# g1mv/density

Measured on NVIDIA H100. Metric: chameleon_encode_input_GBps, higher is better.
Workload: dtype u32

## Files before the change

### density_b200/csrc/chameleon_encode.cu

```cuda
#include <cstdio>
#include "common.cuh"
#include "encode_internal.cuh"

namespace dns {
namespace cham {

constexpr int FP_THREADS = 1024;
constexpr int FP_QPT = 4;
constexpr int TILE_Q = FP_THREADS * FP_QPT;
constexpr int SIDE_N = 8192;
constexpr uint32_t SIDE_EMPTY = 0xFFFFFFFFu;

constexpr int CLS_N = 32;
constexpr int CLS_CAP = 128;

constexpr uint32_t R_TOUCHED = 1u << 12, R_SLOW = 1u << 13, R_FIRST = 1u << 14;

struct FlagSmem {
    uint16_t tab[65536];
    uint32_t vbit[2048];
    uint32_t conf[2048];
    uint32_t side[SIDE_N];
    uint2 rec[TILE_Q];
    uint16_t cls_list[CLS_N][CLS_CAP];
// ... 30 lines not shown
        const uint32_t q = qs[pos];
        const uint32_t p = hash_prod(q);
        const uint32_t hh = valid ? prod_hash(p) : 0x10000u + lane;
        const uint32_t ff = prod_fp(p, q);
        uint32_t cur = 0; bool touched = false;
        if (valid) { cur = S.tab[hh]; touched = cur != 0 || bit_test(S.vbit, hh); }
        const uint32_t grp = __match_any_sync(0xFFFFFFFFu, hh);
        const uint32_t lower = grp & lanemask_lt();
        const int pl = lower ? 31 - __clz(lower) : 0;
        const uint32_t fprev = __shfl_sync(0xFFFFFFFFu, ff, pl);
        const bool hit = valid && (lower ? (fprev == ff) : (touched && cur == ff));
        const bool is_last = (grp & lanemask_gt()) == 0;
        if (valid && is_last && (lower || !hit)) {
            S.tab[hh] = (uint16_t)ff;
            if (ff == 0) atomicOr(&S.vbit[hh >> 5], 1u << (hh & 31));
        }
        const uint32_t fb = __ballot_sync(0xFFFFFFFFu, hit);
        if (lane == 0) S.sigw[c] = fb;
        append_unres(valid && !lower && !touched, run_q0 + pos, hh, ff, &S.unres_count, unres_run);
        __syncwarp();
    }
}

__global__ void __launch_bounds__(FP_THREADS, 1)
cham_flag_pass(const uint32_t* __restrict__ in, uint64_t nquads, uint32_t tiles_total, uint32_t nruns,
               uint32_t* __restrict__ sigw_g,
               uint2* __restrict__ unres,
               uint32_t* __restrict__ unres_count,
               uint32_t* __restrict__ final_tab,
               const uint8_t* __restrict__ copymap,
               const Status* __restrict__ gate)
{
    if (gate && !(gate->nonquiet && !gate->converged)) return;
    extern __shared__ __align__(16) unsigned char smem_raw[];
    FlagSmem& S = *reinterpret_cast<FlagSmem*>(smem_raw);
    const uint32_t tid = threadIdx.x, lane = tid & 31, warp = tid >> 5;
    const uint32_t run = blockIdx.x;
    const uint64_t t_begin = (uint64_t)run * tiles_total / nruns;
    const uint64_t t_end = (uint64_t)(run + 1) * tiles_total / nruns;
    uint2* __restrict__ unres_run = unres + (size_t)run * 65536;
    const uint32_t pos0 = warp * 128 + lane;
    const uint32_t ntile_run = (uint32_t)(t_end - t_begin);
    const uint64_t q_begin = t_begin * TILE_Q;
    const uint64_t q_end64 = (t_end * TILE_Q < nquads) ? t_end * TILE_Q : nquads;
    const uint32_t run_quads = q_begin < q_end64 ? (uint32_t)(q_end64 - q_begin) : 0u;
    const uint32_t* __restrict__ rin = in + q_begin;
    uint32_t* __restrict__ rsig = sigw_g + t_begin * (TILE_Q / 32);
    const uint8_t* __restrict__ rcm = copymap ? copymap + t_begin * 64 : nullptr;

    {
        uint4 z = make_uint4(0, 0, 0, 0);
        uint4* t4 = reinterpret_cast<uint4*>(S.tab);
        #pragma unroll 1
        for (uint32_t i = tid; i < 65536 * 2 / 16; i += FP_THREADS) t4[i] = z;
        #pragma unroll 1
        for (uint32_t i = tid; i < 2048; i += FP_THREADS) { S.vbit[i] = 0; S.conf[i] = 0; }
        #pragma unroll 1
        for (uint32_t i = tid; i < SIDE_N; i += FP_THREADS) S.side[i] = SIDE_EMPTY;
        if (tid < CLS_N) S.cls_count[tid] = 0;
        if (tid == 0) { S.unres_count = 0; S.cls_overflow = 0; S.nrec = 0; }
    }
    __syncthreads();

    uint32_t nxt[FP_QPT];
#pragma unroll
    for (int j = 0; j < FP_QPT; ++j) nxt[j] = (pos0 + 32 * j < run_quads) ? ld_stream_u32(rin + pos0 + 32 * j) : 0u;

#ifdef DNS_PHASE_TIMING
    long long ph[8] = {0, 0, 0, 0, 0, 0, 0, 0}, tprev = clock64();
#define DNS_PH(k) { long long tn = clock64(); ph[k] += tn - tprev; tprev = tn; }
#else
#define DNS_PH(k)
#endif
    #pragma unroll 1
    for (uint32_t lt = 0; lt < ntile_run; ++lt) {
        uint32_t q[FP_QPT], h[FP_QPT], f[FP_QPT];
        const uint32_t run_q0 = lt * TILE_Q;
        const uint32_t left = run_q0 < run_quads ? run_quads - run_q0 : 0u;
        const uint32_t rem = left < (uint32_t)TILE_Q ? left : (uint32_t)TILE_Q;
#pragma unroll
        for (int j = 0; j < FP_QPT; ++j) q[j] = nxt[j];
        {
            const uint32_t nleft = left > (uint32_t)TILE_Q ? left - TILE_Q : 0u;
            const uint32_t* __restrict__ np = rin + run_q0 + TILE_Q + pos0;
#pragma unroll
            for (int j = 0; j < FP_QPT; ++j) nxt[j] = (pos0 + 32 * j < nleft) ? ld_stream_u32(np + 32 * j) : 0u;
        }

        uint32_t actmask = 0;
        {
            uint32_t cp = 0;
            if (rcm) cp = (rcm[lt * 64 + warp * 2] ? 1u : 0u) | (rcm[lt * 64 + warp * 2 + 1] ? 2u : 0u);
#pragma unroll
            for (int j = 0; j < FP_QPT; ++j)
                if (pos0 + 32 * j < rem && !((cp >> (j >> 1)) & 1u)) actmask |= 1u << j;
        }
        uint32_t missmask = 0;
        {
            uint32_t old[FP_QPT], tch = 0;
#pragma unroll
            for (int j = 0; j < FP_QPT; ++j) {
                const uint32_t p = hash_prod(q[j]);
                h[j] = prod_hash(p);
                f[j] = prod_fp(p, q[j]);
                old[j] = S.tab[h[j]];
            }
            uint32_t mb[FP_QPT], tot = 0;
#pragma unroll
            for (int j = 0; j < FP_QPT; ++j) {
                bool touched = old[j] != 0;
                if (!touched) touched = bit_test(S.vbit, h[j]);
                if (touched) tch |= 1u << j;
                const bool miss = ((actmask >> j) & 1u) && !(touched && old[j] == f[j]);
                if (miss) missmask |= 1u << j;
                mb[j] = __ballot_sync(0xFFFFFFFFu, miss);
                tot += __popc(mb[j]);
            }
            if (tot) {
                uint32_t base = 0;
                if (lane == 0) base = atomicAdd(&S.nrec, tot);
                base = __shfl_sync(0xFFFFFFFFu, base, 0);
#pragma unroll
                for (int j = 0; j < FP_QPT; ++j) {
                    if (missmask & (1u << j))
                        S.rec[base + __popc(mb[j] & lanemask_lt())] =
                            make_uint2(h[j] | (f[j] << 16), (pos0 + 32 * j) | ((tch >> j) & 1u ? R_TOUCHED : 0u) | (old[j] << 16));
                    base += __popc(mb[j]);
                }
            }
        }
        __syncthreads();
        DNS_PH(0)
        const uint32_t nmiss = S.nrec;

        #pragma unroll 1
        for (uint32_t i = tid; i < nmiss; i += FP_THREADS) {
            const uint2 r = S.rec[i];
            const uint32_t hh = r.x & 0xFFFFu;
            S.tab[hh] = (uint16_t)(r.x >> 16);
            atomicMin(&S.side[hh & (SIDE_N - 1)], ((r.y & 0xFFFu) << 16) | hh);
        }
        __syncthreads();
        DNS_PH(1)

#pragma unroll
        for (int j = 0; j < FP_QPT; ++j) {
            const uint32_t pos = pos0 + 32 * j;
            bool ok = false;
            if (((actmask >> j) & 1u) && !(missmask & (1u << j))) {
                ok = S.tab[h[j]] == f[j];
                if (!ok) {
                    const uint32_t slot = S.side[h[j] & (SIDE_N - 1)];
                    if ((slot & 0xFFFFu) == h[j] && pos < (slot >> 16)) {
                        ok = true;
                    } else {
                        const uint32_t idx = atomicAdd(&S.nrec, 1u);
                        S.rec[idx] = make_uint2(h[j] | (f[j] << 16), pos | R_TOUCHED | (f[j] << 16));
                        const uint32_t c = h[j] >> 11;
                        const uint32_t k = atomicAdd(&S.cls_count[c], 1u);
                        if (k < CLS_CAP) S.cls_list[c][k] = (uint16_t)idx; else S.cls_overflow = 1;
                        atomicOr(&S.conf[h[j] >> 5], 1u << (h[j] & 31));
                    }
                }
            }
            const uint32_t fb = __ballot_sync(0xFFFFFFFFu, ok);
            if (lane == 0) S.sigw[warp * 4 + j] = fb;
        }
        #pragma unroll 1
        for (uint32_t i = tid; i < nmiss; i += FP_THREADS) {
            const uint2 r = S.rec[i];
            const uint32_t hh = r.x & 0xFFFFu;
            const uint32_t slot = S.side[hh & (SIDE_N - 1)];
            const uint32_t w = S.tab[hh];
            uint32_t y = r.y;
            if ((slot & 0xFFFFu) != hh || w != (r.x >> 16)) {
                y |= R_SLOW;
                atomicOr(&S.conf[hh >> 5], 1u << (hh & 31));
            } else if (slot == (((r.y & 0xFFFu) << 16) | hh)) {
                y |= R_FIRST;
            }
            if (y != r.y) S.rec[i].y = y;
        }
        __syncthreads();
        DNS_PH(2)

        #pragma unroll 1
        for (uint32_t i = tid; i < nmiss; i += FP_THREADS) {
            const uint2 r = S.rec[i];
            const uint32_t hh = r.x & 0xFFFFu;
            uint32_t y = r.y;
            if (!(y & R_SLOW) && bit_test(S.conf, hh)) { y |= R_SLOW; S.rec[i].y = y; }
            if (y & R_SLOW) {
                const uint32_t c = hh >> 11;
                const uint32_t k = atomicAdd(&S.cls_count[c], 1u);
                if (k < CLS_CAP) S.cls_list[c][k] = (uint16_t)i; else S.cls_overflow = 1;
            } else if (!(y & R_FIRST)) {
                const uint32_t pos = y & 0xFFFu;
                atomicOr(&S.sigw[pos >> 5], 1u << (pos & 31));
            }
            S.side[hh & (SIDE_N - 1)] = SIDE_EMPTY;
        }
        __syncthreads();
        DNS_PH(3)

        S.conf[tid] = 0; S.conf[tid + FP_THREADS] = 0;
        if (S.cls_overflow) {
            #pragma unroll 1
            for (uint32_t i = tid; i < nmiss; i += FP_THREADS) {
                const uint2 r = S.rec[i];
                S.tab[r.x & 0xFFFFu] = (uint16_t)(r.y >> 16);
            }
            if (tid < CLS_N) S.cls_count[tid] = 0;
            __syncthreads();
            uint32_t* qs = reinterpret_cast<uint32_t*>(S.rec);
#pragma unroll
            for (int j = 0; j < FP_QPT; ++j) qs[pos0 + 32 * j] = q[j];
            if (tid == 0) { S.nrec = 0; S.cls_overflow = 0; }
            __syncthreads();
            if (warp == 0) tile_in_order(S, qs, rem, run_q0, unres_run, rcm ? rcm + lt * 64 : nullptr);
        } else {
            #pragma unroll 1
            for (uint32_t base = warp * 32; base < nmiss; base += FP_THREADS) {
                const uint32_t i = base + lane;
                uint2 r = make_uint2(0, 0);
                if (i < nmiss) r = S.rec[i];
                const uint32_t hh = r.x & 0xFFFFu;
                const bool first = (i < nmiss) && (r.y & (R_FIRST | R_SLOW)) == R_FIRST;
                if (first && (r.x >> 16) == 0) atomicOr(&S.vbit[hh >> 5], 1u << (hh & 31));
                append_unres(first && !(r.y & R_TOUCHED), run_q0 + (r.y & 0xFFFu), hh, r.x >> 16, &S.unres_count, unres_run);
            }
            const uint32_t n = S.cls_count[warp];
            const uint16_t* __restrict__ lst = S.cls_list[warp];
            #pragma unroll 1
            for (uint32_t base = 0; base < n; base += 32) {
                const uint32_t i = base + lane;
                const bool valid = i < n;
                uint32_t pos = 0, hh = 0xFFFFFFFFu, ff = 0, oldv = 0; bool touched = false;
                if (valid) {
                    const uint2 d = S.rec[lst[i]];
                    hh = d.x & 0xFFFFu; ff = d.x >> 16; pos = d.y & 0xFFFu; touched = (d.y & R_TOUCHED) != 0; oldv = d.y >> 16;
                }
                int best = -1; uint32_t bestf = 0; bool later = false;
                #pragma unroll 1
                for (uint32_t k = 0; k < n; ++k) {
                    const uint2 dk = S.rec[lst[k]];
                    const uint32_t pk = dk.y & 0xFFFu;
                    if ((dk.x & 0xFFFFu) == hh) {
                        if (pk < pos && (int)pk > best) { best = (int)pk; bestf = dk.x >> 16; }
                        later |= pk > pos;
                    }
                }
                const bool hit = valid && (best >= 0 ? (bestf == ff) : (touched && oldv == ff));
                if (hit) atomicOr(&S.sigw[pos >> 5], 1u << (pos & 31));
                if (valid && !later) {
                    S.tab[hh] = (uint16_t)ff;
                    if (ff == 0) atomicOr(&S.vbit[hh >> 5], 1u << (hh & 31));
                }
                append_unres(valid && best < 0 && !touched, run_q0 + pos, hh, ff, &S.unres_count, unres_run);
            }
            __syncwarp();
            if (lane == 0) S.cls_count[warp] = 0;
            if (tid == 0) S.nrec = 0;
        }
        __syncthreads();
        DNS_PH(4)

        if (tid < TILE_Q / 32) rsig[lt * (TILE_Q / 32) + tid] = S.sigw[tid];
    }

#ifdef DNS_PHASE_TIMING
    if (tid == 0 && run == 77) { const long long nt = (long long)ntile_run;
        printf("run %u tiles %lld cycles/tile: A %lld B %lld C %lld D %lld F %lld  total %lld\n", run, nt,
               ph[0] / nt, ph[1] / nt, ph[2] / nt, ph[3] / nt, ph[4] / nt, (ph[0] + ph[1] + ph[2] + ph[3] + ph[4]) / nt); }
#endif
    #pragma unroll 1
    for (uint32_t i = tid; i < 65536; i += FP_THREADS) {
        uint32_t v = S.tab[i];
        uint32_t tch = (v != 0 || bit_test(S.vbit, i)) ? 0x10000u : 0u;
        final_tab[(size_t)run * 65536 + i] = v | tch;
    }
    if (tid == 0) unres_count[run] = S.unres_count < 65536u ? S.unres_count : 65536u;
}

constexpr int F6_THREADS = 512, F6_QPT = 8;
constexpr int F6_NW = F6_THREADS / 32, F6_WQ = 32 * F6_QPT;
static_assert(F6_THREADS * F6_QPT == TILE_Q, "tile geometry");
constexpr int F6_MB_SLOTS = 4096, F6_MB_CAP = 4;
constexpr int F6_SEC_SLOTS = 64, F6_SEC_CAP = 16;
#ifdef DNS_PHASE_TIMING
__device__ long long g_f6_ph[8];
#define F6_PH(k) { if (threadIdx.x == 0 && blockIdx.x == 77) { long long tn = clock64(); g_f6_ph[k] += tn - f6_tprev; f6_tprev = tn; } }
#define F6_PH_DECL long long f6_tprev = clock64();
#else
#define F6_PH(k)
#define F6_PH_DECL
#endif
constexpr uint32_t F6_TOUCHED = 1u << 12, F6_DROPPED = 1u << 13;
struct Flag6Smem {
    uint16_t tab[65536];
    uint32_t vbit[2048];
    uint2 rec[TILE_Q];
    union {
        uint16_t mb[F6_MB_SLOTS][F6_MB_CAP];
        uint2 dense[TILE_Q];
    };
    uint32_t mbcnt[2][F6_MB_SLOTS / 4];
    __align__(16) uint32_t sec[F6_SEC_SLOTS][F6_SEC_CAP];
    uint32_t seccnt[2][F6_SEC_SLOTS];
    uint32_t sigw[2][TILE_Q / 32];
    uint32_t cnt[32];
    uint32_t unres_count;
    uint32_t overflow;
};
static_assert(sizeof(Flag6Smem) <= 227 * 1024, "flag pass shared memory");

__device__ __forceinline__ void f6_append_unres(bool pred, uint32_t qidx_in_run, uint32_t hf, uint32_t* s_count, uint2* __restrict__ unres_run) {
    const uint32_t m = __ballot_sync(0xFFFFFFFFu, pred);
    if (m == 0) return;
    uint32_t base = 0;
    if ((threadIdx.x & 31) == 0) base = atomicAdd(s_count, (uint32_t)__popc(m));
    base = __shfl_sync(0xFFFFFFFFu, base, 0);
    if (pred) {
        const uint32_t idx = base + __popc(m & lanemask_lt());
        if (idx < 65536u) unres_run[idx] = make_uint2(qidx_in_run, hf);
    }
}

__device__ __noinline__ void f6_replay(Flag6Smem& S, uint32_t buf, uint32_t run_q0, uint2* __restrict__ unres_run) {
    const uint32_t lane = threadIdx.x & 31;
    const uint32_t c = lane < (uint32_t)F6_NW ? S.cnt[lane] : 0u;
    uint32_t incl = c;
#pragma unroll
    for (int d = 1; d < 32; d <<= 1) { const uint32_t t = __shfl_up_sync(0xFFFFFFFFu, incl, d); if ((int)lane >= d) incl += t; }
    const uint32_t excl = incl - c;
    const uint32_t n = __shfl_sync(0xFFFFFFFFu, incl, 31);
    #pragma unroll 1
    for (uint32_t i0 = 0; i0 < n; i0 += 32) {
        const uint32_t i = i0 + lane;
        uint32_t w = 0;
#pragma unroll
        for (int b = 16; b >= 1; b >>= 1) { const uint32_t t = __shfl_sync(0xFFFFFFFFu, incl, (w + b - 1) & 31); if (t <= i) w += b; }
        const uint32_t e = __shfl_sync(0xFFFFFFFFu, excl, w & 31);
        if (i < n) {
            const uint2 r = S.rec[w * F6_WQ + (i - e)];
            S.dense[i] = r;
            S.tab[r.x & 0xFFFFu] = (uint16_t)(r.y >> 16);
        }
    }
    __syncwarp();
    #pragma unroll 1
    for (uint32_t i0 = 0; i0 < n; i0 += 32) {
        const uint32_t i = i0 + lane;
        const bool valid = i < n;
        uint2 r = make_uint2(0, 0);
        if (valid) r = S.dense[i];
        const uint32_t hh = r.x & 0xFFFFu, ff = r.x >> 16, pos = r.y & 0xFFFu;
        uint32_t cur = 0;
        if (valid) cur = S.tab[hh];
        const uint32_t grp = __match_any_sync(0xFFFFFFFFu, valid ? hh : 0x10000u + lane);
        const uint32_t lower = grp & lanemask_lt();
        const uint32_t fprev = __shfl_sync(0xFFFFFFFFu, ff, lower ? 31 - __clz(lower) : 0);
        bool touched = true, hit;
        if (lower) hit = fprev == ff;
        else {
            if (cur == 0) touched = bit_test(S.vbit, hh);
            hit = touched && cur == ff;
        }
        if (valid && (grp & lanemask_gt()) == 0) {
            S.tab[hh] = (uint16_t)ff;
            if (ff == 0) atomicOr(&S.vbit[hh >> 5], 1u << (hh & 31));
        }
        if (valid && hit) atomicOr(&S.sigw[buf][pos >> 5], 1u << (pos & 31));
        f6_append_unres(valid && !touched, run_q0 + pos, r.x, &S.unres_count, unres_run);
        __syncwarp();
    }
}

template <bool GENERIC>
__device__ __forceinline__ void f6_tile(Flag6Smem& S, const uint32_t (&q)[F6_QPT], uint32_t validmask, uint32_t buf, uint32_t run_q0,
                                        uint2* __restrict__ unres_run) {
    const uint32_t tid = threadIdx.x, lane = tid & 31, warp = tid >> 5;
    const uint32_t pos0 = warp * F6_WQ + lane;
    uint32_t h[F6_QPT], f[F6_QPT], old[F6_QPT];
    uint32_t missmask = 0;
    F6_PH_DECL
#pragma unroll
    for (int k = 0; k < F6_MB_SLOTS / 4 / F6_THREADS; ++k) S.mbcnt[buf ^ 1u][tid + k * F6_THREADS] = 0;
    if (tid < F6_SEC_SLOTS) S.seccnt[buf ^ 1u][tid] = 0;
#pragma unroll
    for (int j = 0; j < F6_QPT; ++j) {
        const uint32_t p = hash_prod(q[j]);
        h[j] = prod_hash(p);
        f[j] = prod_fp(p, q[j]);
        old[j] = S.tab[h[j]];
    }
    uint32_t fmin = f[0];
#pragma unroll
    for (int j = 0; j < F6_QPT; ++j) {
        bool miss = old[j] != f[j];
        if (GENERIC) miss = miss && ((validmask >> j) & 1u);
        if (miss) missmask |= 1u << j;
        fmin = min(fmin, f[j]);
    }
    if (fmin == 0) {
#pragma unroll
        for (int j = 0; j < F6_QPT; ++j)
            if (f[j] == 0 && old[j] == 0 && (!GENERIC || ((validmask >> j) & 1u)) && !bit_test(S.vbit, h[j])) missmask |= 1u << j;
    }
    __syncthreads();
    F6_PH(0)
#pragma unroll
    for (int j = 0; j < F6_QPT; ++j)
        if (missmask & (1u << j)) S.tab[h[j]] = (uint16_t)f[j];
    __syncthreads();
    F6_PH(1)
    uint32_t clean[F6_QPT], base = 0;
    uint2* __restrict__ myrec = S.rec + warp * F6_WQ;
#pragma unroll
    for (int j = 0; j < F6_QPT; ++j) {
        bool dirty = (missmask >> j) & 1u;
        if (!dirty) dirty = S.tab[h[j]] != f[j];
        if (GENERIC) dirty = dirty && ((validmask >> j) & 1u);
        const uint32_t db = __ballot_sync(0xFFFFFFFFu, dirty);
        clean[j] = GENERIC ? __ballot_sync(0xFFFFFFFFu, !dirty && ((validmask >> j) & 1u)) : ~db;
        if (dirty) myrec[base + __popc(db & lanemask_lt())] = make_uint2(h[j] | (f[j] << 16), (pos0 + 32 * j) | (old[j] << 16));
        base += __popc(db);
    }
    if (lane == 0) {
#pragma unroll
        for (int j = 0; j < F6_QPT; j += 4)
            *reinterpret_cast<uint4*>(&S.sigw[buf][warp * F6_QPT + j]) = make_uint4(clean[j], clean[j + 1], clean[j + 2], clean[j + 3]);
        S.cnt[warp] = base;
    }
    __syncwarp();
    uint2 r0 = make_uint2(0, 0);
    bool drop0 = false;
    {
        uint32_t carry_x = 0xFFFFFFFFu, carry_pos = 0xFFFFFFFFu;
        #pragma unroll 1
        for (uint32_t i0 = 0; i0 < base; i0 += 32) {
            const uint32_t i = i0 + lane;
            const bool valid = i < base;
            uint2 r = make_uint2(0xFFFFFFFFu, 0);
            if (valid) {
                r = myrec[i];
                if ((r.y >> 16) != 0 || bit_test(S.vbit, r.x & 0xFFFFu)) r.y |= F6_TOUCHED;
            }
            uint32_t px = __shfl_up_sync(0xFFFFFFFFu, r.x, 1), ppos = __shfl_up_sync(0xFFFFFFFFu, r.y & 0xFFFu, 1);
            if (lane == 0) { px = carry_x; ppos = carry_pos; }
            const bool drop = valid && px == r.x && ppos + 1 == (r.y & 0xFFFu);
            carry_x = __shfl_sync(0xFFFFFFFFu, r.x, 31); carry_pos = __shfl_sync(0xFFFFFFFFu, r.y & 0xFFFu, 31);
            if (i0 == 0) { r0 = r; drop0 = drop; }
            if (drop) {
                const uint32_t pos = r.y & 0xFFFu;
                atomicOr(&S.sigw[buf][pos >> 5], 1u << (pos & 31));
                if (i0) myrec[i].y = r.y | F6_DROPPED;
            } else if (valid) {
                if (i0 && (r.y & F6_TOUCHED)) myrec[i].y = r.y;
                const uint32_t hh = r.x & 0xFFFFu, slot = hh & (F6_MB_SLOTS - 1), sh = (slot & 3u) * 8u;
                const uint32_t k = (atomicAdd(&S.mbcnt[buf][slot >> 2], 1u << sh) >> sh) & 0xFFu;
                if (k < (uint32_t)F6_MB_CAP) S.mb[slot][k] = (uint16_t)(((hh >> 12) << 12) | (warp * F6_WQ + i));
                else {
                    const uint32_t s2 = slot & (F6_SEC_SLOTS - 1);
                    const uint32_t k2 = atomicAdd(&S.seccnt[buf][s2], 1u);
                    if (k2 < (uint32_t)F6_SEC_CAP) S.sec[s2][k2] = (hh << 12) | (warp * F6_WQ + i);
                    else S.overflow = 1;
                }
            }
        }
    }
    __syncthreads();
    F6_PH(2)
#ifdef DNS_PHASE_TIMING
    if (threadIdx.x == 0 && blockIdx.x == 77) { g_f6_ph[6] += S.overflow; uint32_t tot = 0; for (int w = 0; w < 32; ++w) tot += S.cnt[w]; g_f6_ph[7] += tot; }
#endif
    if (S.overflow) {
        if (warp == 0) f6_replay(S, buf, run_q0, unres_run);
    } else {
        #pragma unroll 1
        for (uint32_t i0 = 0; i0 < base; i0 += 32) {
            const uint32_t i = i0 + lane;
            bool valid = i < base;
            uint2 r = r0;
            if (i0) r = valid ? myrec[i] : make_uint2(0, 0);
            if (i0 ? (r.y & F6_DROPPED) != 0 : drop0) valid = false;
            const uint32_t hh = r.x & 0xFFFFu, ff = r.x >> 16, pos = r.y & 0xFFFu, slot = hh & (F6_MB_SLOTS - 1);
            const uint32_t myidx = warp * F6_WQ + i;
            bool later = false, hit = false, unres = false;
            if (valid) {
                const uint32_t n = (S.mbcnt[buf][slot >> 2] >> ((slot & 3u) * 8u)) & 0xFFu;
                const uint2 e2 = *reinterpret_cast<const uint2*>(&S.mb[slot][0]);
                const uint32_t me = ((hh >> 12) << 12) | myidx;
                int best = -1;
#pragma unroll
                for (int t = 0; t < F6_MB_CAP; ++t) {
                    const uint32_t e = ((t & 2) ? e2.y : e2.x) >> ((t & 1) * 16) & 0xFFFFu;
                    if ((uint32_t)t < n && ((e ^ me) >> 12) == 0) {
                        if (e < me) best = max(best, (int)(e & 0xFFFu));
                        later |= e > me;
                    }
                }
                if (n > (uint32_t)F6_MB_CAP) {
                    const uint32_t s2 = slot & (F6_SEC_SLOTS - 1);
                    const uint32_t n2 = S.seccnt[buf][s2];
                    const uint32_t mine = (hh << 12) | myidx;
                    #pragma unroll 1
                    for (uint32_t t4 = 0; t4 < n2; t4 += 4) {
                        const uint4 e4 = *reinterpret_cast<const uint4*>(&S.sec[s2][t4]);
                        const uint32_t ev[4] = {e4.x, e4.y, e4.z, e4.w};
#pragma unroll
                        for (int t = 0; t < 4; ++t) {
                            const uint32_t e = ev[t];
                            if (t4 + t < n2 && ((e ^ mine) & 0xFFFFF000u) == 0) {
                                if (e < mine) best = max(best, (int)(e & 0xFFFu));
                                later |= e > mine;
                            }
                        }
                    }
                }
                if (best >= 0) hit = (S.rec[best].x >> 16) == ff;
                else if (r.y & F6_TOUCHED) hit = (r.y >> 16) == ff;
                else unres = true;
                if (!later) {
                    S.tab[hh] = (uint16_t)ff;
                    if (ff == 0) atomicOr(&S.vbit[hh >> 5], 1u << (hh & 31));
                }
                if (hit) atomicOr(&S.sigw[buf][pos >> 5], 1u << (pos & 31));
            }
            f6_append_unres(unres, run_q0 + pos, r.x, &S.unres_count, unres_run);
        }
    }
    __syncthreads();
    F6_PH(3)
}

__global__ void __launch_bounds__(F6_THREADS, 1)
cham_flag_pass6(const uint32_t* __restrict__ in, uint64_t nquads, uint32_t tiles_total, uint32_t nruns,
                uint32_t* __restrict__ sigw_g, uint2* __restrict__ unres, uint32_t* __restrict__ unres_count,
                uint32_t* __restrict__ final_tab, const uint8_t* __restrict__ copymap, const Status* __restrict__ gate)
{
    if (gate && !(gate->nonquiet && !gate->converged)) return;
    extern __shared__ __align__(16) unsigned char smem_raw[];
    Flag6Smem& S = *reinterpret_cast<Flag6Smem*>(smem_raw);
    const uint32_t tid = threadIdx.x, lane = tid & 31, warp = tid >> 5;
    const uint32_t run = blockIdx.x;
    const uint64_t t_begin = (uint64_t)run * tiles_total / nruns;
    const uint64_t t_end = (uint64_t)(run + 1) * tiles_total / nruns;
    uint2* __restrict__ unres_run = unres + (size_t)run * 65536;
    const uint32_t pos0 = warp * F6_WQ + lane;
    const uint32_t ntile_run = (uint32_t)(t_end - t_begin);
    const uint64_t q_begin = t_begin * TILE_Q;
    const uint64_t q_end64 = (t_end * TILE_Q < nquads) ? t_end * TILE_Q : nquads;
    const uint32_t run_quads = q_begin < q_end64 ? (uint32_t)(q_end64 - q_begin) : 0u;
    const uint32_t* __restrict__ rin = in + q_begin;
    uint32_t* __restrict__ rsig = sigw_g + t_begin * (TILE_Q / 32);
    const uint8_t* __restrict__ rcm = copymap ? copymap + t_begin * 64 : nullptr;
    {
        const uint4 z = make_uint4(0, 0, 0, 0);
        uint4* t4 = reinterpret_cast<uint4*>(S.tab);
        #pragma unroll 1
        for (uint32_t i = tid; i < 65536 * 2 / 16; i += F6_THREADS) t4[i] = z;
        #pragma unroll 1
        for (uint32_t i = tid; i < 2048; i += F6_THREADS) S.vbit[i] = 0;
        #pragma unroll 1
        for (uint32_t i = tid; i < F6_MB_SLOTS / 4; i += F6_THREADS) { S.mbcnt[0][i] = 0; S.mbcnt[1][i] = 0; }
        if (tid < F6_SEC_SLOTS) { S.seccnt[0][tid] = 0; S.seccnt[1][tid] = 0; }
        if (tid == 0) { S.unres_count = 0; S.overflow = 0; }
    }
    __syncthreads();
    uint32_t nxt[F6_QPT];
#pragma unroll
    for (int j = 0; j < F6_QPT; ++j) nxt[j] = (pos0 + 32 * j < run_quads) ? ld_stream_u32(rin + pos0 + 32 * j) : 0u;
    #pragma unroll 1
    for (uint32_t lt = 0; lt < ntile_run; ++lt) {
        uint32_t q[F6_QPT];
        const uint32_t run_q0 = lt * TILE_Q;
        const uint32_t left = run_q0 < run_quads ? run_quads - run_q0 : 0u;
        const uint32_t buf = lt & 1u;
#pragma unroll
        for (int j = 0; j < F6_QPT; ++j) q[j] = nxt[j];
        {
            const uint32_t nleft = left > (uint32_t)TILE_Q ? left - TILE_Q : 0u;
            const uint32_t* __restrict__ np = rin + run_q0 + TILE_Q + pos0;
            if (nleft >= (uint32_t)TILE_Q) {
#pragma unroll
                for (int j = 0; j < F6_QPT; ++j) nxt[j] = ld_stream_u32(np + 32 * j);
            } else {
#pragma unroll
                for (int j = 0; j < F6_QPT; ++j) nxt[j] = (pos0 + 32 * j < nleft) ? ld_stream_u32(np + 32 * j) : 0u;
            }
        }
        if (left >= (uint32_t)TILE_Q && !rcm) {
            f6_tile<false>(S, q, (1u << F6_QPT) - 1u, buf, run_q0, unres_run);
        } else {
            uint32_t validmask = 0, cp = 0;
            if (rcm) {
#pragma unroll
                for (int b = 0; b < F6_WQ / 64; ++b) cp |= (rcm[lt * 64 + warp * (F6_WQ / 64) + b] ? 1u : 0u) << b;
            }
#pragma unroll
            for (int j = 0; j < F6_QPT; ++j)
                if (pos0 + 32 * j < left && !((cp >> (j >> 1)) & 1u)) validmask |= 1u << j;
            f6_tile<true>(S, q, validmask, buf, run_q0, unres_run);
        }
        if (tid < TILE_Q / 32) rsig[lt * (TILE_Q / 32) + tid] = S.sigw[buf][tid];
        if (tid == 0) S.overflow = 0;
    }
    #pragma unroll 1
    for (uint32_t i = tid; i < 65536; i += F6_THREADS) {
        const uint32_t v = S.tab[i];
        const uint32_t tch = (v != 0 || bit_test(S.vbit, i)) ? 0x10000u : 0u;
        final_tab[(size_t)run * 65536 + i] = v | tch;
    }
    if (tid == 0) unres_count[run] = S.unres_count < 65536u ? S.unres_count : 65536u;
#ifdef DNS_PHASE_TIMING
    if (tid == 0 && run == 77 && ntile_run) { const long long nt = ntile_run;
        printf("f6 run %u tiles %lld cycles/tile: A %lld B %lld C+deposit %lld D+S4 %lld  overflow tiles %lld dirty/tile %lld\n", run, nt, g_f6_ph[0] / nt, g_f6_ph[1] / nt,
               g_f6_ph[2] / nt, g_f6_ph[3] / nt, g_f6_ph[6], g_f6_ph[7] / nt);
        for (int k = 0; k < 8; ++k) g_f6_ph[k] = 0; }
#endif
}

__device__ __forceinline__ bool gate_open(const Status* g) { return !g || (g->nonquiet && !g->converged); }

__global__ void cham_carry_scan(const uint32_t* __restrict__ final_tab, const uint32_t* __restrict__ init, int init_untouched,
                                uint32_t nruns, uint32_t* __restrict__ carry, uint32_t* __restrict__ table_out,
                                const Status* __restrict__ gate = nullptr) {
    if (!gate_open(gate)) return;
    uint32_t hb = blockIdx.x * blockDim.x + threadIdx.x;
    if (hb >= 65536) return;
    uint32_t c = init ? init[hb] : ((hb == 0 && !init_untouched) ? 0x10000u : 0u);
    for (uint32_t r = 0; r < nruns; ++r) {
        if (carry) carry[(size_t)r * 65536 + hb] = c;
        uint32_t v = final_tab[(size_t)r * 65536 + hb];
        if (v & 0x10000u) c = v;
    }
    if (table_out) table_out[hb] = c;
}

__global__ void cham_resolve(const uint2* __restrict__ unres, const uint32_t* __restrict__ unres_count,
                             const uint32_t* __restrict__ carry, uint32_t tiles_total, uint32_t nruns,
                             uint32_t* __restrict__ sigw_g, const Status* __restrict__ gate = nullptr) {
    if (!gate_open(gate)) return;
    const uint32_t run = blockIdx.y;
    const uint32_t n = unres_count[run];
    const uint64_t run_q0 = ((uint64_t)run * tiles_total / nruns) * TILE_Q;
    for (uint32_t i = blockIdx.x * blockDim.x + threadIdx.x; i < n; i += gridDim.x * blockDim.x) {
        uint2 e = unres[(size_t)run * 65536 + i];
        uint32_t c = carry[(size_t)run * 65536 + (e.y & 0xFFFFu)];
        if ((c & 0x10000u) && (c & 0xFFFFu) == (e.y >> 16)) {
            uint64_t gq = run_q0 + e.x;
            atomicOr(&sigw_g[gq >> 5], 1u << (gq & 31));
        }
    }
}

struct ProtSmem {
    uint16_t tab[65536];
    uint32_t vbit[2048];
};

__global__ void __launch_bounds__(1024, 1)
cham_protected_pass(const uint32_t* __restrict__ in, uint64_t nbytes, const Status* __restrict__ status, int only_if_nonquiet,
                    uint32_t* __restrict__ sigw_g, uint8_t* __restrict__ copymap) {
    if (only_if_nonquiet && !(status->nonquiet && !status->converged)) return;
    extern __shared__ __align__(16) unsigned char smem_raw[];
    ProtSmem& S = *reinterpret_cast<ProtSmem*>(smem_raw);
    const uint32_t tid = threadIdx.x, lane = tid & 31;
    {
        uint4 z = make_uint4(0, 0, 0, 0);
        uint4* t4 = reinterpret_cast<uint4*>(S.tab);
        for (uint32_t i = tid; i < 65536 * 2 / 16; i += blockDim.x) t4[i] = z;
        for (uint32_t i = tid; i < 2048; i += blockDim.x) S.vbit[i] = (i == 0) ? 1u : 0u;
    }
    __syncthreads();
    if (tid >= 32) return;

    const uint64_t nquads = nbytes / 4;
    const uint64_t nblocks = (nbytes + 255) / 256;
    Protection ps; ps.init();
    uint32_t n0 = 0, n1 = 0;
    if (nblocks) {
        if (lane < nquads) n0 = in[lane];
        if (32 + lane < nquads) n1 = in[32 + lane];
    }
    for (uint64_t b = 0; b < nblocks; ++b) {
        const uint32_t q0 = n0, q1 = n1;
        {
            uint64_t g = (b + 1) * 64 + lane;
            n0 = (b + 1 < nblocks && g < nquads) ? in[g] : 0u;
            n1 = (b + 1 < nblocks && g + 32 < nquads) ? in[g + 32] : 0u;
        }
        const uint64_t bq0 = b * 64;
        const uint32_t nq = (uint32_t)((nquads - bq0 < 64) ? (nquads - bq0) : 64);
        if (ps.revert_to_copy()) {
            if (lane == 0) { copymap[b] = 1; sigw_g[2 * b] = 0; sigw_g[2 * b + 1] = 0; }
            ps.decay();
            continue;
        }
        uint32_t sig[2];
#pragma unroll
        for (int half = 0; half < 2; ++half) {
            const uint32_t q = half ? q1 : q0;
            const bool valid = half * 32 + lane < nq;
            const uint32_t p = hash_prod(q);
            uint32_t hh = valid ? prod_hash(p) : 0x10000u + lane;
            const uint32_t ff = prod_fp(p, q);
            uint32_t cur = 0; bool touched = false;
            if (valid) { cur = S.tab[hh]; touched = cur != 0 || bit_test(S.vbit, hh); }
            const uint32_t grp = __match_any_sync(0xFFFFFFFFu, hh);
            const uint32_t lower = grp & lanemask_lt();
            const int pl = lower ? 31 - __clz(lower) : 0;
            const uint32_t fprev = __shfl_sync(0xFFFFFFFFu, ff, pl);
            const bool hit = valid && (lower ? (fprev == ff) : (touched && cur == ff));
            const bool is_last = (grp & lanemask_gt()) == 0;
            if (valid && is_last && (lower || !hit)) {
                S.tab[hh] = (uint16_t)ff;
                if (ff == 0) atomicOr(&S.vbit[hh >> 5], 1u << (hh & 31));
            }
            sig[half] = __ballot_sync(0xFFFFFFFFu, hit);
            __syncwarp();
        }
        if (lane == 0) { copymap[b] = 0; sigw_g[2 * b] = sig[0]; sigw_g[2 * b + 1] = sig[1]; }
        const uint32_t hits = __popc(sig[0]) + __popc(sig[1]);
        const uint32_t tailb = (b == nblocks - 1) ? (uint32_t)(nbytes & 3) : 0u;
        const uint32_t out_sz = 8 + 4 * nq - 2 * hits + tailb;
        ps.update(out_sz >= 256);
    }
}

constexpr int PSEG = 256;

__device__ __forceinline__ uint32_t prot_pack(const Protection& ps) { return ps.copy_penalty | (ps.copy_penalty_start << 8) | (ps.previous_incompressible << 16); }
__device__ __forceinline__ void prot_walk(Protection& ps, const uint8_t* __restrict__ inc, uint64_t b0, uint64_t b1, uint8_t* __restrict__ cm) {
    for (uint64_t b = b0; b < b1; ++b) {
        if (ps.revert_to_copy()) { cm[b] = 1; ps.decay(); }
        else { cm[b] = 0; ps.update(__ldcg(&inc[b]) != 0); }
    }
}
constexpr int PROT_ROUNDS = 48, PROT_FAST_ROUNDS = 4;
constexpr int PI_THREADS = 1024;

constexpr uint32_t PC_NS = 10, PC_NP = 10, PC_NC = 2 * PC_NS * PC_NP, PC_ESC = 0xFFFFu, PC_GROUP = 128;
__host__ __device__ __forceinline__ size_t prot_table_elems(uint64_t nseg) {
    const uint64_t ngrp = (nseg + PC_GROUP - 1) / PC_GROUP;
    return (size_t)(2 * (ngrp + 2) + nseg * PC_NC + ngrp * PC_NC + 64);
}
__device__ __forceinline__ void pc_decode(uint32_t c, Protection& ps) {
    ps.copy_penalty = c % PC_NP; ps.copy_penalty_start = (c / PC_NP) % PC_NS + 1u; ps.previous_incompressible = c / (PC_NP * PC_NS);
}
__device__ __forceinline__ uint32_t pc_encode(const Protection& ps) {
    if (ps.copy_penalty >= PC_NP || ps.copy_penalty_start < 1u || ps.copy_penalty_start > PC_NS) return PC_ESC;
    return (ps.previous_incompressible * PC_NS + (ps.copy_penalty_start - 1u)) * PC_NP + ps.copy_penalty;
}

__device__ __forceinline__ void grid_barrier(unsigned int* counter, unsigned int nctas, unsigned int& epoch) {
    __syncthreads();
    if (threadIdx.x == 0) {
        __threadfence();
        atomicAdd(counter, 1u);
        const unsigned int target = (epoch + 1) * nctas;
        while (atomicAdd(counter, 0u) < target) { __nanosleep(64); }
        __threadfence();
    }
    ++epoch;
    __syncthreads();
}

__device__ unsigned long long g_prot_dbg[16][2];

__global__ void __launch_bounds__(PI_THREADS)
prot_iterate(const uint32_t* __restrict__ sigw_g, uint64_t nbytes, uint64_t nblocks, uint32_t nseg, Status* __restrict__ st, int it,
             uint8_t* __restrict__ inc, uint8_t* __restrict__ cm_old, uint8_t* __restrict__ cm_new,
             uint32_t* __restrict__ in_state, uint32_t* __restrict__ out_state, uint16_t* __restrict__ ptab) {
    if (!gate_open(st)) return;
    __shared__ uint32_t s_state[1024], s_in[1024];
    __shared__ uint8_t s_inc[PSEG], s_cm[PSEG];
    __shared__ uint32_t s_cur, s_redo;
    const uint32_t tid = threadIdx.x;
    const uint64_t gtid = (uint64_t)blockIdx.x * PI_THREADS + tid, gsz = (uint64_t)gridDim.x * PI_THREADS;
// ... 834 lines not shown
```

Measured before the change: 423.9.

## Parallelize overflow replay across all warps by partitioning hash space

The overflow fallback replay, which previously ran serially on warp 0 over all dirty records, now runs on all 16 warps. Each warp owns the hash bucket class hh>>12 and scans every warp's records, staging its own entries into a per-warp buffer and processing them in batches of 32. Table restores are first done in parallel followed by a block barrier. The drop-detection carry initialisation is also changed to explicitly exclude index 0, and the timing probe loop bound is fixed. The change relies on the overflow path being hit often enough to matter, and adds per-warp staging and full rescans of the records.

After: 448.7, median of 6. 1.06x the previous value.

```diff
diff --git a/density_b200/csrc/chameleon_encode.cu b/density_b200/csrc/chameleon_encode.cu
--- a/density_b200/csrc/chameleon_encode.cu
+++ b/density_b200/csrc/chameleon_encode.cu
@@ -356,7 +356,7 @@
     uint2 rec[TILE_Q];
     union {
         uint16_t mb[F6_MB_SLOTS][F6_MB_CAP];
-        uint2 dense[TILE_Q];
+        uint2 stage[F6_NW][64];
     };
     uint32_t mbcnt[2][F6_MB_SLOTS / 4];
     __align__(16) uint32_t sec[F6_SEC_SLOTS][F6_SEC_CAP];
@@ -380,54 +380,74 @@
     }
 }
 
+static_assert(F6_NW == 16, "one warp per bucket class hash >> 12");
+__device__ __forceinline__ void f6_replay_step(Flag6Smem& S, const uint2* stage, uint32_t n, uint32_t buf, uint32_t run_q0,
+                                               uint2* __restrict__ unres_run) {
+    const uint32_t lane = threadIdx.x & 31;
+    const bool valid = lane < n;
+    uint2 r = make_uint2(0, 0);
+    if (valid) r = stage[lane];
+    const uint32_t hh = r.x & 0xFFFFu, ff = r.x >> 16, pos = r.y & 0xFFFu;
+    uint32_t cur = 0;
+    if (valid) cur = S.tab[hh];
+    const uint32_t grp = __match_any_sync(0xFFFFFFFFu, valid ? hh : 0x10000u + lane);
+    const uint32_t lower = grp & lanemask_lt();
+    const uint32_t fprev = __shfl_sync(0xFFFFFFFFu, ff, lower ? 31 - __clz(lower) : 0);
+    bool touched = true, hit;
+    if (lower) hit = fprev == ff;
+    else {
+        if (cur == 0) touched = bit_test(S.vbit, hh);
+        hit = touched && cur == ff;
+    }
+    if (valid && (grp & lanemask_gt()) == 0) {
+        S.tab[hh] = (uint16_t)ff;
+        if (ff == 0) atomicOr(&S.vbit[hh >> 5], 1u << (hh & 31));
+    }
+    if (valid && hit) atomicOr(&S.sigw[buf][pos >> 5], 1u << (pos & 31));
+    f6_append_unres(valid && !touched, run_q0 + pos, r.x, &S.unres_count, unres_run);
+    __syncwarp();
+}
+
 __device__ __noinline__ void f6_replay(Flag6Smem& S, uint32_t buf, uint32_t run_q0, uint2* __restrict__ unres_run) {
-    const uint32_t lane = threadIdx.x & 31;
-    const uint32_t c = lane < (uint32_t)F6_NW ? S.cnt[lane] : 0u;
-    uint32_t incl = c;
-#pragma unroll
-    for (int d = 1; d < 32; d <<= 1) { const uint32_t t = __shfl_up_sync(0xFFFFFFFFu, incl, d); if ((int)lane >= d) incl += t; }
-    const uint32_t excl = incl - c;
-    const uint32_t n = __shfl_sync(0xFFFFFFFFu, incl, 31);
+    const uint32_t lane = threadIdx.x & 31, warp = threadIdx.x >> 5;
+    {
+        const uint32_t n = S.cnt[warp];
+        const uint2* __restrict__ myrec = S.rec + warp * F6_WQ;
+        #pragma unroll 1
+        for (uint32_t i = lane; i < n; i += 32) {
+            const uint2 r = myrec[i];
+            S.tab[r.x & 0xFFFFu] = (uint16_t)(r.y >> 16);
+        }
+    }
+    __syncthreads();
+    uint2* __restrict__ stage = S.stage[warp];
+    uint32_t ns = 0;
     #pragma unroll 1
-    for (uint32_t i0 = 0; i0 < n; i0 += 32) {
-        const uint32_t i = i0 + lane;
-        uint32_t w = 0;
-#pragma unroll
-        for (int b = 16; b >= 1; b >>= 1) { const uint32_t t = __shfl_sync(0xFFFFFFFFu, incl, (w + b - 1) & 31); if (t <= i) w += b; }
-        const uint32_t e = __shfl_sync(0xFFFFFFFFu, excl, w & 31);
-        if (i < n) {
-            const uint2 r = S.rec[w * F6_WQ + (i - e)];
-            S.dense[i] = r;
-            S.tab[r.x & 0xFFFFu] = (uint16_t)(r.y >> 16);
+    for (uint32_t w = 0; w < (uint32_t)F6_NW; ++w) {
+        const uint32_t n = S.cnt[w];
+        const uint2* __restrict__ rg = S.rec + w * F6_WQ;
+        #pragma unroll 1
+        for (uint32_t i0 = 0; i0 < n; i0 += 32) {
+            const uint32_t i = i0 + lane;
+            uint2 r = make_uint2(0, 0);
+            if (i < n) r = rg[i];
+            const bool mine = i < n && ((r.x & 0xFFFFu) >> 12) == warp;
+            const uint32_t m = __ballot_sync(0xFFFFFFFFu, mine);
+            if (mine) stage[ns + __popc(m & lanemask_lt())] = r;
+            ns += __popc(m);
+            if (ns >= 32) {
+                __syncwarp();
+                f6_replay_step(S, stage, 32, buf, run_q0, unres_run);
+                const uint2 rest = stage[32 + lane];
+                __syncwarp();
+                if (lane < ns - 32) stage[lane] = rest;
+                ns -= 32;
+                __syncwarp();
+            }
         }
     }
     __syncwarp();
-    #pragma unroll 1
-    for (uint32_t i0 = 0; i0 < n; i0 += 32) {
-        const uint32_t i = i0 + lane;
-        const bool valid = i < n;
-        uint2 r = make_uint2(0, 0);
-        if (valid) r = S.dense[i];
-        const uint32_t hh = r.x & 0xFFFFu, ff = r.x >> 16, pos = r.y & 0xFFFu;
-        uint32_t cur = 0;
-        if (valid) cur = S.tab[hh];
-        const uint32_t grp = __match_any_sync(0xFFFFFFFFu, valid ? hh : 0x10000u + lane);
-        const uint32_t lower = grp & lanemask_lt();
-        const uint32_t fprev = __shfl_sync(0xFFFFFFFFu, ff, lower ? 31 - __clz(lower) : 0);
-        bool touched = true, hit;
-        if (lower) hit = fprev == ff;
-        else {
-            if (cur == 0) touched = bit_test(S.vbit, hh);
-            hit = touched && cur == ff;
-        }
-        if (valid && (grp & lanemask_gt()) == 0) {
-            S.tab[hh] = (uint16_t)ff;
-            if (ff == 0) atomicOr(&S.vbit[hh >> 5], 1u << (hh & 31));
-        }
-        if (valid && hit) atomicOr(&S.sigw[buf][pos >> 5], 1u << (pos & 31));
-        f6_append_unres(valid && !touched, run_q0 + pos, r.x, &S.unres_count, unres_run);
-        __syncwarp();
-    }
+    if (ns) f6_replay_step(S, stage, ns, buf, run_q0, unres_run);
 }
 
 template <bool GENERIC>
@@ -490,7 +510,7 @@
     uint2 r0 = make_uint2(0, 0);
     bool drop0 = false;
     {
-        uint32_t carry_x = 0xFFFFFFFFu, carry_pos = 0xFFFFFFFFu;
+        uint32_t carry_x = 0, carry_pos = 0;
         #pragma unroll 1
         for (uint32_t i0 = 0; i0 < base; i0 += 32) {
             const uint32_t i = i0 + lane;
@@ -502,7 +522,7 @@
             }
             uint32_t px = __shfl_up_sync(0xFFFFFFFFu, r.x, 1), ppos = __shfl_up_sync(0xFFFFFFFFu, r.y & 0xFFFu, 1);
             if (lane == 0) { px = carry_x; ppos = carry_pos; }
-            const bool drop = valid && px == r.x && ppos + 1 == (r.y & 0xFFFu);
+            const bool drop = valid && i != 0 && px == r.x && ppos + 1 == (r.y & 0xFFFu);
             carry_x = __shfl_sync(0xFFFFFFFFu, r.x, 31); carry_pos = __shfl_sync(0xFFFFFFFFu, r.y & 0xFFFu, 31);
             if (i0 == 0) { r0 = r; drop0 = drop; }
             if (drop) {
@@ -526,10 +546,10 @@
     __syncthreads();
     F6_PH(2)
 #ifdef DNS_PHASE_TIMING
-    if (threadIdx.x == 0 && blockIdx.x == 77) { g_f6_ph[6] += S.overflow; uint32_t tot = 0; for (int w = 0; w < 32; ++w) tot += S.cnt[w]; g_f6_ph[7] += tot; }
+    if (threadIdx.x == 0 && blockIdx.x == 77) { g_f6_ph[6] += S.overflow; uint32_t tot = 0; for (int w = 0; w < F6_NW; ++w) tot += S.cnt[w]; g_f6_ph[7] += tot; }
 #endif
     if (S.overflow) {
-        if (warp == 0) f6_replay(S, buf, run_q0, unres_run);
+        f6_replay(S, buf, run_q0, unres_run);
     } else {
         #pragma unroll 1
         for (uint32_t i0 = 0; i0 < base; i0 += 32) {
```
